# kaspanet/rusty-kaspa

Hardware: AMD Instinct MI355X
Metric: sig-verifies/sec (higher is better)
Workload: dtype u256; 1 GPU; schnorr-verify-1M; tuples_per_gpu=1048576, invalid_permille=0, parallelism=single

## Files before the change

### rusty_kaspa_amd/csrc/kv_secp_device.h

```cpp
#ifndef KV_SECP_DEVICE_H
#define KV_SECP_DEVICE_H

#ifndef KV_HOST_TEST
#include <hip/hip_runtime.h>
#endif
#include <stdint.h>

namespace kv {

#ifdef KV_GROUP_INLINE
#define KV_GROUP_ATTR inline
#else
#define KV_GROUP_ATTR __noinline__
#endif
#if defined(KV_GROUP_INLINE) || defined(KV_DOUBLE_INLINE)
#define KV_DOUBLE_ATTR inline
#else
#define KV_DOUBLE_ATTR __noinline__
#endif

typedef uint64_t u64;
typedef uint32_t u32;
typedef unsigned __int128 u128;


struct fe {
  u64 n[4];
};

#define KV_P0 0xFFFFFFFEFFFFFC2FULL
#define KV_P1 0xFFFFFFFFFFFFFFFFULL
#define KV_PC 0x1000003D1ULL

__device__ __forceinline__ u64 addc(u64 a, u64 b, u64 &carry) {
  u128 t = (u128)a + b + carry;
  carry = (u64)(t >> 64);
  return (u64)t;
}

__device__ __forceinline__ u64 subb(u64 a, u64 b, u64 &borrow) {
  u128 t = (u128)a - b - borrow;
  borrow = (u64)(t >> 64) & 1;
  return (u64)t;
}

__device__ __forceinline__ void fe_norm_once(fe &a) {
  u64 ge = (a.n[3] == KV_P1) & (a.n[2] == KV_P1) & (a.n[1] == KV_P1) &
           (a.n[0] >= KV_P0);
  u64 mask = 0 - ge;
  u64 borrow = 0;
  a.n[0] = subb(a.n[0], KV_P0 & mask, borrow);
  a.n[1] = subb(a.n[1], KV_P1 & mask, borrow);
  a.n[2] = subb(a.n[2], KV_P1 & mask, borrow);
  a.n[3] = subb(a.n[3], KV_P1 & mask, borrow);
}

__device__ __forceinline__ void fe_mul_inner(u64 t[8], const u64 *an, const u64 *bn) {
#pragma unroll
  for (int i = 0; i < 8; i++) t[i] = 0;
#pragma unroll
  for (int i = 0; i < 4; i++) {
    u64 carry = 0;
#pragma unroll
    for (int j = 0; j < 4; j++) {
      u128 cur = (u128)an[i] * bn[j] + t[i + j] + carry;
      t[i + j] = (u64)cur;
      carry = (u64)(cur >> 64);
    }
    t[i + 4] = carry;
  }
}

__device__ __forceinline__ void fe_reduce8(fe &r, const u64 t[8]) {
  u128 c = (u128)t[0] + (u128)t[4] * KV_PC;
  u64 s0 = (u64)c;
  c = (c >> 64) + t[1] + (u128)t[5] * KV_PC;
  u64 s1 = (u64)c;
  c = (c >> 64) + t[2] + (u128)t[6] * KV_PC;
  u64 s2 = (u64)c;
  c = (c >> 64) + t[3] + (u128)t[7] * KV_PC;
  u64 s3 = (u64)c;
  u64 s4 = (u64)(c >> 64);
  c = (u128)s0 + (u128)s4 * KV_PC;
  r.n[0] = (u64)c;
  c = (c >> 64) + s1;
  r.n[1] = (u64)c;
  c = (c >> 64) + s2;
  r.n[2] = (u64)c;
  c = (c >> 64) + s3;
  r.n[3] = (u64)c;
  if ((u64)(c >> 64)) {
    c = (u128)r.n[0] + KV_PC;
    r.n[0] = (u64)c;
    u64 cc = (u64)(c >> 64);
    r.n[1] += cc;
  }
  fe_norm_once(r);
}

__device__ __forceinline__ void fe_mul(fe &r, const fe &a, const fe &b) {
  u64 t[8];
  fe_mul_inner(t, a.n, b.n);
  fe_reduce8(r, t);
}


#define KV26_M ((u32)0x3FFFFFF)
#define KV26_R0 ((u64)0x3D10)

struct fe26 {
#ifdef KV_FE26_ALIGN
  alignas(16) u32 l[10];
#else
  u32 l[10];
#endif
};

#ifdef KV_HOST_TEST
#include <assert.h>
#define KV26_CHECK_MUL_IN(a)                                                   \
  do {                                                                         \
    for (int _i = 0; _i < 10; _i++) assert((a).l[_i] <= (1u << 30));           \
  } while (0)
#else
#define KV26_CHECK_MUL_IN(a)
#endif

__device__ __forceinline__ void fe26_reduce19(fe26 &r, const u64 t[19]) {
  u32 u[11];
  u64 c = t[9] >> 26;
#pragma unroll
  for (int k = 0; k < 9; k++) {
    u64 d = t[k + 10] + c;
    u[k] = (u32)d & KV26_M;
    c = d >> 26;
  }
  u[9] = (u32)c & KV26_M;
  u[10] = (u32)(c >> 26);
  u64 W = ((u64)u[9] << 10) + (u64)u[10] * KV26_R0 + ((u64)u[10] << 36);
  u32 w0 = (u32)W & KV26_M, w1 = (u32)(W >> 26);
  u64 cc = 0;
#pragma unroll
  for (int k = 0; k < 10; k++) {
    u64 d = (k == 9 ? (t[9] & KV26_M) : t[k]) + cc + (u64)u[k] * KV26_R0;
    if (k >= 1) d += (u64)u[k - 1] << 10;
    if (k == 0) d += (u64)w0 * KV26_R0;
    if (k == 1) d += ((u64)w0 << 10) + (u64)w1 * KV26_R0;
    if (k == 2) d += (u64)w1 << 10;
    r.l[k] = (u32)d & KV26_M;
    cc = d >> 26;
  }
#ifdef KV_HOST_TEST
  assert(u[10] <= (1u << 8) && W < ((u64)1 << 45) && cc < (1u << 15));
#endif
  u32 x = (r.l[9] >> 22) + ((u32)cc << 4);
  r.l[9] &= 0x3FFFFF;
  r.l[0] += x * 977u;
  r.l[1] += (x << 6) + (r.l[0] >> 26);
  r.l[0] &= KV26_M;
  r.l[2] += r.l[1] >> 26;
  r.l[1] &= KV26_M;
}

__device__ __forceinline__ void fe26_mul_inner(u64 t[19], const fe26 &a,
                                               const fe26 &b) {
  KV26_CHECK_MUL_IN(a);
  KV26_CHECK_MUL_IN(b);
#pragma unroll
  for (int k = 0; k < 19; k++) t[k] = 0;
#pragma unroll
  for (int i = 0; i < 10; i++)
#pragma unroll
    for (int j = 0; j < 10; j++) t[i + j] += (u64)a.l[i] * b.l[j];

}

__device__ __forceinline__ void fe26_sqr_inner(u64 t[19], const fe26 &a) {
  KV26_CHECK_MUL_IN(a);
  u32 d[9];
#pragma unroll
  for (int i = 0; i < 9; i++) d[i] = a.l[i] << 1;
#pragma unroll
  for (int k = 0; k < 19; k++) t[k] = 0;
#pragma unroll
  for (int i = 0; i < 10; i++) {
    t[2 * i] += (u64)a.l[i] * a.l[i];
#pragma unroll
    for (int j = i + 1; j < 10; j++) t[i + j] += (u64)d[i] * a.l[j];
  }
}

__device__ __forceinline__ void fe26_mul(fe26 &r, const fe26 &a, const fe26 &b) {
  u64 t[19];
  fe26_mul_inner(t, a, b);
  fe26_reduce19(r, t);
}

__device__ __forceinline__ void fe26_sqr(fe26 &r, const fe26 &a) {
  u64 t[19];
  fe26_sqr_inner(t, a);
  fe26_reduce19(r, t);
}

__device__ __forceinline__ void fe26_add(fe26 &r, const fe26 &a, const fe26 &b) {
#pragma unroll
  for (int i = 0; i < 10; i++) r.l[i] = a.l[i] + b.l[i];
}

__device__ __forceinline__ void fe26_neg(fe26 &r, const fe26 &a, u32 m) {
  r.l[0] = (u32)(0x3FFFC2FUL * 2 * (m + 1)) - a.l[0];
  r.l[1] = (u32)(0x3FFFFBFUL * 2 * (m + 1)) - a.l[1];
#pragma unroll
  for (int i = 2; i < 9; i++) r.l[i] = (u32)(0x3FFFFFFUL * 2 * (m + 1)) - a.l[i];
  r.l[9] = (u32)(0x3FFFFFUL * 2 * (m + 1)) - a.l[9];
}

__device__ __forceinline__ void fe26_mul_int(fe26 &r, u32 k) {
#pragma unroll
  for (int i = 0; i < 10; i++) r.l[i] *= k;
}

__device__ __forceinline__ void fe26_cmov(fe26 &r, const fe26 &a, u32 cond) {
  u32 mask = 0 - cond;
#pragma unroll
  for (int i = 0; i < 10; i++) r.l[i] = (r.l[i] & ~mask) | (a.l[i] & mask);
}

__device__ __forceinline__ void fe26_norm_weak(fe26 &a) {
  u32 c = 0;
#pragma unroll
  for (int i = 0; i < 10; i++) {
    u32 d = a.l[i] + c;
    a.l[i] = d & KV26_M;
    c = d >> 26;
  }
  a.l[0] += c * (u32)KV26_R0;
  a.l[1] += c << 10;
  u32 x = a.l[9] >> 22;
  a.l[9] &= 0x3FFFFF;
  a.l[0] += x * 977u;
  a.l[1] += x << 6;
}

__device__ __forceinline__ void fe26_normalize(fe26 &a) {
  fe26_norm_weak(a);
#pragma unroll 1
  for (int pass = 0; pass < 3; pass++) {
    u32 c = 0;
#pragma unroll
    for (int i = 0; i < 10; i++) {
      u32 d = a.l[i] + c;
      a.l[i] = d & KV26_M;
      c = d >> 26;
    }
    u32 x = (a.l[9] >> 22) | (c << 4);
    a.l[9] &= 0x3FFFFF;
    a.l[0] += x * 977u;
    a.l[1] += x << 6;
  }
  u32 t[10];
  u64 d = (u64)a.l[0] + 977u;
  t[0] = (u32)(d & KV26_M);
  d = (d >> 26) + a.l[1] + (1u << 6);
  t[1] = (u32)(d & KV26_M);
#pragma unroll
  for (int i = 2; i < 10; i++) {
    d = (d >> 26) + a.l[i];
    t[i] = (u32)(d & KV26_M);
  }
  u32 ge = (u32)(t[9] >> 22) & 1;
  t[9] &= 0x3FFFFF;
  u32 mask = 0 - ge;
#pragma unroll
  for (int i = 0; i < 10; i++) a.l[i] = (a.l[i] & ~mask) | (t[i] & mask);
}

__device__ __forceinline__ int fe26_is_zero(const fe26 &a) {
  fe26 t = a;
  fe26_normalize(t);
  u32 z = 0;
#pragma unroll
  for (int i = 0; i < 10; i++) z |= t.l[i];
  return z == 0;
}

__device__ __forceinline__ int fe26_eq(const fe26 &a, const fe26 &b) {
  fe26 ta = a, tb = b;
  fe26_normalize(ta);
  fe26_normalize(tb);
  u32 d = 0;
#pragma unroll
  for (int i = 0; i < 10; i++) d |= ta.l[i] ^ tb.l[i];
  return d == 0;
}

__device__ __forceinline__ int fe26_normalizes_to_zero(const fe26 &a) {
#ifdef KV_HOST_TEST
  for (int _i = 0; _i < 10; _i++) assert(a.l[_i] < (1u << 31));
#endif
  u32 l[10];
  u32 c = 0;
#pragma unroll
  for (int i = 0; i < 10; i++) {
    u32 d = a.l[i] + c;
    l[i] = d & KV26_M;
    c = d >> 26;
  }
  u32 x = l[9] >> 22;
  l[9] &= 0x3FFFFF;
  l[0] += c * (u32)KV26_R0 + x * 977u;
  l[1] += (c << 10) + (x << 6) + (l[0] >> 26);
  l[0] &= KV26_M;
  l[2] += l[1] >> 26;
  l[1] &= KV26_M;
  u32 z0 = l[0] | l[1] | l[2] | l[9];
  u32 z1 = (l[0] ^ 0x3D0u) & (l[1] ^ 0x40u) & l[2] & (l[9] ^ 0x3C00000u);
#pragma unroll
  for (int i = 3; i < 9; i++) {
    z0 |= l[i];
    z1 &= l[i];
  }
  return (z0 == 0) | (z1 == KV26_M);
}

__device__ __forceinline__ void fe26_from_fe(fe26 &r, const fe &a) {
#pragma unroll
  for (int i = 0; i < 10; i++) {
    int bit = 26 * i;
    int w = bit >> 6, sh = bit & 63;
    u64 v = a.n[w] >> sh;
    if (sh > 38 && w < 3) v |= a.n[w + 1] << (64 - sh);
    r.l[i] = (u32)(v & KV26_M);
  }
  r.l[9] &= 0x3FFFFF;
}

__device__ __forceinline__ void fe26_to_fe(fe &r, const fe26 &a) {
  r.n[0] = (u64)a.l[0] | ((u64)a.l[1] << 26) | ((u64)a.l[2] << 52);
  r.n[1] = ((u64)a.l[2] >> 12) | ((u64)a.l[3] << 14) | ((u64)a.l[4] << 40);
  r.n[2] = ((u64)a.l[4] >> 24) | ((u64)a.l[5] << 2) | ((u64)a.l[6] << 28) |
           ((u64)a.l[7] << 54);
  r.n[3] = ((u64)a.l[7] >> 10) | ((u64)a.l[8] << 16) | ((u64)a.l[9] << 42);
}


struct sc {
  u64 d[4];
};

#define KV_N0 0xBFD25E8CD0364141ULL
#define KV_N1 0xBAAEDCE6AF48A03BULL
#define KV_N2 0xFFFFFFFFFFFFFFFEULL
#define KV_N3 0xFFFFFFFFFFFFFFFFULL
#define KV_NC0 0x402DA1732FC9BEBFULL
#define KV_NC1 0x4551231950B75FC4ULL
#define KV_NC2 1ULL

__device__ __forceinline__ int sc_gte_n(const sc &a) {
  if (a.d[3] > KV_N3) return 1;
  if (a.d[3] < KV_N3) return 0;
  if (a.d[2] > KV_N2) return 1;
  if (a.d[2] < KV_N2) return 0;
  if (a.d[1] > KV_N1) return 1;
  if (a.d[1] < KV_N1) return 0;
  return a.d[0] >= KV_N0;
}

__device__ __forceinline__ void sc_sub_n(sc &a) {
  u64 borrow = 0;
  a.d[0] = subb(a.d[0], KV_N0, borrow);
  a.d[1] = subb(a.d[1], KV_N1, borrow);
  a.d[2] = subb(a.d[2], KV_N2, borrow);
  a.d[3] = subb(a.d[3], KV_N3, borrow);
}

__device__ __forceinline__ int sc_is_zero(const sc &a) {
  return (a.d[0] | a.d[1] | a.d[2] | a.d[3]) == 0;
}

__device__ __forceinline__ int sc_from_be(sc &r, const uint8_t b[32]) {
#pragma unroll
  for (int i = 0; i < 4; i++) {
    u64 w = 0;
#pragma unroll
    for (int j = 0; j < 8; j++) w = (w << 8) | b[8 * (3 - i) + j];
    r.d[i] = w;
  }
  int ov = sc_gte_n(r);
  if (ov) sc_sub_n(r);
  return ov;
}

__device__ __forceinline__ void sc_neg(sc &r, const sc &a) {
  u64 is_zero = sc_is_zero(a);
  u64 borrow = 0;
  r.d[0] = subb(KV_N0, a.d[0], borrow);
  r.d[1] = subb(KV_N1, a.d[1], borrow);
  r.d[2] = subb(KV_N2, a.d[2], borrow);
  r.d[3] = subb(KV_N3, a.d[3], borrow);
  u64 mask = 0 - is_zero;
  r.d[0] &= ~mask;
  r.d[1] &= ~mask;
  r.d[2] &= ~mask;
  r.d[3] &= ~mask;
}

__device__ inline void sc_reduce8(sc &r, const u64 tin[8]) {
  const u64 NC[3] = {KV_NC0, KV_NC1, KV_NC2};
  u64 s[7] = {tin[0], tin[1], tin[2], tin[3], 0, 0, 0};
  for (int i = 0; i < 4; i++) {
    u64 carry = 0;
    for (int j = 0; j < 3; j++) {
      u64 lo = tin[4 + i] * NC[j];
      u64 hi = __umul64hi(tin[4 + i], NC[j]);
      u64 c = 0;
      s[i + j] = addc(s[i + j], lo, c);
      u64 c2 = 0;
      s[i + j] = addc(s[i + j], carry, c2);
      carry = hi + c + c2;
    }
    u64 c = 0;
    s[i + 3] = addc(s[i + 3], carry, c);
    for (int k = i + 4; k < 7 && c; k++) s[k] = addc(s[k], 0, c);
  }
  u64 u[5] = {s[0], s[1], s[2], s[3], 0};
  for (int i = 0; i < 3; i++) {
    u64 carry = 0;
    for (int j = 0; j < 3; j++) {
      int pos = i + j;
      u64 lo = s[4 + i] * NC[j];
      u64 hi = __umul64hi(s[4 + i], NC[j]);
      u64 c = 0;
      u[pos] = addc(u[pos], lo, c);
      u64 c2 = 0;
      u[pos] = addc(u[pos], carry, c2);
      carry = hi + c + c2;
    }
    if (i + 3 < 5) {
      u64 c = 0;
      u[i + 3] = addc(u[i + 3], carry, c);
      for (int k = i + 4; k < 5 && c; k++) u[k] = addc(u[k], 0, c);
    }
  }
  u64 w[4] = {u[0], u[1], u[2], u[3]};
  {
    u64 carry = 0;
    for (int j = 0; j < 3; j++) {
      u64 lo = u[4] * NC[j];
      u64 hi = __umul64hi(u[4], NC[j]);
      u64 c = 0;
      w[j] = addc(w[j], lo, c);
      u64 c2 = 0;
      w[j] = addc(w[j], carry, c2);
      carry = hi + c + c2;
    }
    u64 c = 0;
    w[3] = addc(w[3], carry, c);
    if (c) {
      u64 cc = 0;
      w[0] = addc(w[0], NC[0], cc);
      w[1] = addc(w[1], NC[1], cc);
      w[2] = addc(w[2], NC[2], cc);
      w[3] = addc(w[3], 0, cc);
    }
  }
  r.d[0] = w[0]; r.d[1] = w[1]; r.d[2] = w[2]; r.d[3] = w[3];
  while (sc_gte_n(r)) sc_sub_n(r);
}

__device__ inline void sc_mul(sc &r, const sc &a, const sc &b) {
  u64 t[8];
  fe_mul_inner(t, a.d, b.d);
  sc_reduce8(r, t);
}

__device__ KV_GROUP_ATTR void sc_sqrn(sc &r, int n) {
#pragma unroll 1
  for (int i = 0; i < n; i++) sc_mul(r, r, r);
}

__device__ KV_GROUP_ATTR void sc_inv(sc &r, const sc &a) {
  static const uint8_t WIN[33] = {14, 11, 10, 10, 14, 13, 12, 14, 6,  10, 15,
                                  4,  8,  10, 0,  3,  11, 11, 15, 13, 2,  5,
                                  14, 8,  12, 13, 0,  3,  6,  4,  1,  3,  15};
  sc tab[16];
  tab[0] = {{1, 0, 0, 0}};
  tab[1] = a;
#pragma unroll 1
  for (int i = 2; i < 16; i++) sc_mul(tab[i], tab[i - 1], a);
  sc x6, x12, x24, t;
  const sc &x3 = tab[7], &x4 = tab[15];
  t = x3;
  sc_sqrn(t, 3);
  sc_mul(x6, t, x3);
  t = x6;
  sc_sqrn(t, 6);
  sc_mul(x12, t, x6);
  t = x12;
  sc_sqrn(t, 12);
  sc_mul(x24, t, x12);
  t = x24;
  sc_sqrn(t, 24);
  sc_mul(t, t, x24);
  sc x48 = t;
  sc_sqrn(t, 48);
  sc_mul(t, t, x48);
  sc_sqrn(t, 24);
  sc_mul(t, t, x24);
  sc_sqrn(t, 4);
  sc_mul(t, t, x4);
#pragma unroll 1
  for (int i = 0; i < 33; i++) {
    sc_sqrn(t, 4);
    sc m;
    sc_mul(m, t, tab[WIN[i]]);
    t = m;
  }
  r = t;
}


__device__ KV_GROUP_ATTR void fe26_sqrn(fe26 &r, int n) {
#pragma unroll 1
  for (int i = 0; i < n; i++) fe26_sqr(r, r);
}

__device__ KV_GROUP_ATTR void fe26_chain223(fe26 &x223, fe26 &x22, fe26 &x2,
                                            fe26 &x3, const fe26 &a) {
  fe26 t, x11, x44, x88;
  fe26_sqr(t, a);
  fe26_mul(x2, t, a);
  fe26_sqr(t, x2);
  fe26_mul(x3, t, a);
  t = x3;
  fe26_sqrn(t, 3);
  fe26_mul(t, t, x3);
  fe26_sqrn(t, 3);
  fe26_mul(t, t, x3);
  fe26_sqrn(t, 2);
  fe26_mul(x11, t, x2);
  t = x11;
  fe26_sqrn(t, 11);
  fe26_mul(x22, t, x11);
  t = x22;
  fe26_sqrn(t, 22);
  fe26_mul(x44, t, x22);
  t = x44;
  fe26_sqrn(t, 44);
  fe26_mul(x88, t, x44);
  t = x88;
  fe26_sqrn(t, 88);
  fe26_mul(t, t, x88);
  fe26_sqrn(t, 44);
  fe26_mul(t, t, x44);
  fe26_sqrn(t, 3);
  fe26_mul(x223, t, x3);
}

__device__ inline void fe26_inv(fe26 &r, const fe26 &a) {
  fe26 x223, x22, x2, x3, t;
  fe26_chain223(x223, x22, x2, x3, a);
  t = x223;
  fe26_sqrn(t, 23);
  fe26_mul(t, t, x22);
  fe26_sqrn(t, 5);
  fe26_mul(t, t, a);
  fe26_sqrn(t, 3);
  fe26_mul(t, t, x2);
  fe26_sqrn(t, 2);
  fe26_mul(r, t, a);
}

__device__ inline int fe26_sqrt(fe26 &r, const fe26 &a) {
  fe26 x223, x22, x2, x3, t, chk;
  fe26_chain223(x223, x22, x2, x3, a);
  t = x223;
  fe26_sqrn(t, 23);
  fe26_mul(t, t, x22);
  fe26_sqrn(t, 6);
  fe26_mul(t, t, x2);
  fe26_sqrn(t, 2);
  fe26_sqr(chk, t);
  r = t;
  fe26 aa = a;
  return fe26_eq(chk, aa);
}


struct ge {
  fe26 x, y;
};

struct gej {
  fe26 x, y, z;
};

__device__ __forceinline__ void fe26_set_int(fe26 &r, u32 v) {
  r.l[0] = v;
#pragma unroll
  for (int i = 1; i < 10; i++) r.l[i] = 0;
}

__device__ __forceinline__ void gej_set_infinity(gej &r) {
  fe26_set_int(r.x, 1);
  fe26_set_int(r.y, 1);
  fe26_set_int(r.z, 0);
}

__device__ __forceinline__ int gej_is_infinity(const gej &a) {
  return fe26_normalizes_to_zero(a.z);
}

__device__ __forceinline__ void gej_double_impl(gej &r, const gej &a) {
  fe26 A, B, C, D, E, F, t, x4, y2;
  fe26_sqr(A, a.x);
  fe26_sqr(B, a.y);
  fe26_sqr(C, B);
  x4 = a.x;
  fe26_mul_int(x4, 4);
  fe26_mul(D, x4, B);
  E = A;
  fe26_mul_int(E, 3);
  fe26_sqr(F, E);
  fe26 nx, ny, nz, nD;
  fe26_neg(nD, D, 2);
  fe26_add(nx, F, nD);
  fe26_add(nx, nx, nD);
  fe26_norm_weak(nx);
  fe26 nnx;
  fe26_neg(nnx, nx, 2);
  fe26_add(t, D, nnx);
  fe26_mul(t, E, t);
  fe26 C8;
  C8 = C;
  fe26_mul_int(C8, 8);
  fe26 nC8;
  fe26_neg(nC8, C8, 16);
  fe26_add(ny, t, nC8);
  fe26_norm_weak(ny);
  fe26_add(y2, a.y, a.y);
  fe26_mul(nz, y2, a.z);
  r.x = nx;
  r.y = ny;
  r.z = nz;
}

__device__ KV_DOUBLE_ATTR void gej_double(gej &r, const gej &a) {
  gej_double_impl(r, a);
}

__device__ KV_GROUP_ATTR void gej_double4(gej &r, const gej &a) {
  gej t;
  gej_double_impl(t, a);
  gej_double_impl(r, t);
  gej_double_impl(t, r);
  gej_double_impl(r, t);
}

__device__ __forceinline__ void gej_cmov(gej &r, const gej &a, u64 cond) {
  u32 c = (u32)(cond & 1);
  fe26_cmov(r.x, a.x, c);
  fe26_cmov(r.y, a.y, c);
  fe26_cmov(r.z, a.z, c);
}

template <bool ZR>
__device__ __forceinline__ void gej_add_ge_core(gej &r, fe26 &zr, const gej &a,
                                                const ge &b) {
  u64 a_inf = (u64)fe26_normalizes_to_zero(a.z);
  fe26 z1z1, u2, s2, h, hh, i, j, rr, v, t;
  fe26_sqr(z1z1, a.z);
  fe26_mul(s2, b.y, a.z);
  fe26_mul(u2, b.x, z1z1);
  fe26_mul(s2, s2, z1z1);
  fe26 nX, nY;
  fe26_neg(nX, a.x, 2);
  fe26_neg(nY, a.y, 2);
  fe26_add(h, u2, nX);
  fe26_add(rr, s2, nY);
  if (!a_inf && fe26_normalizes_to_zero(h)) {
    if (fe26_normalizes_to_zero(rr)) {
      gej t2;
      gej ain = a;
      fe26_norm_weak(ain.x);
      fe26_norm_weak(ain.y);
      fe26_norm_weak(ain.z);
      gej_double_impl(t2, ain);
      r = t2;
      if (ZR) {
        fe26_add(zr, ain.y, ain.y);
        fe26_norm_weak(zr);
      }
    } else {
      gej_set_infinity(r);
      if (ZR) fe26_set_int(zr, 0);
    }
    return;
  }
  if (ZR) {
    fe26_add(zr, h, h);
    fe26_norm_weak(zr);
  }
  fe26 zz;
  fe26_add(zz, a.z, h);
  fe26_sqr(zz, zz);
  fe26_sqr(hh, h);
  i = hh;
  fe26_mul_int(i, 4);
  fe26_mul(j, h, i);
  fe26_mul(v, a.x, i);
  fe26 nx, ny, nz;
  fe26_sqr(nx, rr);
  fe26_mul_int(nx, 4);
  fe26 nj, nv;
  fe26_neg(nj, j, 2);
  fe26_neg(nv, v, 2);
  fe26_add(nx, nx, nj);
  fe26_add(nx, nx, nv);
  fe26_add(nx, nx, nv);
  fe26_norm_weak(nx);
  fe26 nnx;
  fe26_neg(nnx, nx, 2);
  fe26_add(t, v, nnx);
  fe26_mul(t, rr, t);
  fe26_add(t, t, t);
  fe26 y1j;
  fe26_mul(y1j, a.y, j);
  fe26_add(y1j, y1j, y1j);
  fe26 ny1j;
  fe26_neg(ny1j, y1j, 4);
  fe26_add(ny, t, ny1j);
  fe26_norm_weak(ny);
  fe26 nzz, nhh;
  fe26_neg(nzz, z1z1, 2);
  fe26_neg(nhh, hh, 2);
  fe26_add(nz, zz, nzz);
  fe26_add(nz, nz, nhh);
  fe26_norm_weak(nz);
  fe26 one;
  fe26_set_int(one, 1);
  u32 ci = (u32)(a_inf & 1);
  fe26_cmov(nx, b.x, ci);
  fe26_cmov(ny, b.y, ci);
  fe26_cmov(nz, one, ci);
  r.x = nx;
  r.y = ny;
  r.z = nz;
}

__device__ __forceinline__ void gej_add_ge_impl(gej &r, const gej &a, const ge &b) {
  fe26 unused;
  gej_add_ge_core<false>(r, unused, a, b);
}

__device__ KV_GROUP_ATTR void gej_add_ge(gej &r, const gej &a, const ge &b) {
  gej_add_ge_impl(r, a, b);
}

__device__ KV_GROUP_ATTR void gej_add_ge_zr(gej &r, fe26 &zr, const gej &a,
                                            const ge &b) {
  gej_add_ge_core<true>(r, zr, a, b);
}

__device__ KV_GROUP_ATTR void gej_add(gej &r, const gej &a, const gej &b) {
  u64 a_inf = (u64)fe26_normalizes_to_zero(a.z);
  fe26 z1z1, z2z2, u1, u2, s1, s2, h, i, j, rr, v, t;
  fe26_sqr(z1z1, a.z);
  fe26_sqr(z2z2, b.z);
  fe26_mul(u1, a.x, z2z2);
  fe26_mul(u2, b.x, z1z1);
  fe26_mul(s1, a.y, b.z);
  fe26_mul(s1, s1, z2z2);
  fe26_mul(s2, b.y, a.z);
  fe26_mul(s2, s2, z1z1);
  fe26 nu1, ns1;
  fe26_neg(nu1, u1, 2);
  fe26_neg(ns1, s1, 2);
  fe26_add(h, u2, nu1);
  fe26_add(rr, s2, ns1);
  if (!a_inf && !fe26_normalizes_to_zero(b.z) && fe26_normalizes_to_zero(h)) {
    if (fe26_normalizes_to_zero(rr)) {
      gej t2;
      gej ain = a;
      fe26_norm_weak(ain.x);
      fe26_norm_weak(ain.y);
      fe26_norm_weak(ain.z);
      gej_double_impl(t2, ain);
      r = t2;
    } else {
      gej_set_infinity(r);
    }
    return;
  }
  fe26 zz;
  fe26_add(zz, a.z, b.z);
  fe26_sqr(zz, zz);
  fe26_sqr(i, h);
  fe26_mul_int(i, 4);
  fe26_mul(j, h, i);
  fe26_mul(v, u1, i);
  fe26 nx, ny, nz;
  fe26_sqr(nx, rr);
  fe26_mul_int(nx, 4);
  fe26 nj, nv;
  fe26_neg(nj, j, 2);
  fe26_neg(nv, v, 2);
  fe26_add(nx, nx, nj);
  fe26_add(nx, nx, nv);
  fe26_add(nx, nx, nv);
  fe26_norm_weak(nx);
  fe26 nnx;
  fe26_neg(nnx, nx, 2);
  fe26_add(t, v, nnx);
  fe26_mul(t, rr, t);
  fe26_add(t, t, t);
  fe26 s1j;
  fe26_mul(s1j, s1, j);
  fe26_add(s1j, s1j, s1j);
  fe26 ns1j;
  fe26_neg(ns1j, s1j, 4);
  fe26_add(ny, t, ns1j);
  fe26_norm_weak(ny);
  fe26 nzz1, nzz2;
  fe26_neg(nzz1, z1z1, 2);
  fe26_neg(nzz2, z2z2, 2);
  fe26_add(zz, zz, nzz1);
  fe26_add(zz, zz, nzz2);
  fe26_mul(nz, zz, h);
  u32 ci = (u32)(a_inf & 1);
  fe26_cmov(nx, b.x, ci);
  fe26_cmov(ny, b.y, ci);
  fe26_cmov(nz, b.z, ci);
  r.x = nx;
  r.y = ny;
  r.z = nz;
}

}

#endif
```

### rusty_kaspa_amd/csrc/kv_secp_kernels.hip

```cpp
#include "kv_hash_device.h"
#include "kv_secp_device.h"

namespace kv {

__device__ __constant__ static const uint32_t BIP340_CHALLENGE_MID[8] = {
    0x9cecba11u, 0x23925381u, 0x11679112u, 0xd1627e0fu,
    0x97c87550u, 0x003cc765u, 0x90f61164u, 0x33e9b66au};

enum : uint8_t {
  KVS_VALID = 0,
  KVS_INVALID = 1,
  KVS_BAD_PUBKEY = 2,
  KVS_BAD_SIG = 3,
};

__device__ __forceinline__ void fe_from_be(fe &r, const uint8_t b[32]) {
#pragma unroll
  for (int i = 0; i < 4; i++) {
    u64 w = 0;
#pragma unroll
    for (int j = 0; j < 8; j++) w = (w << 8) | b[8 * (3 - i) + j];
    r.n[i] = w;
  }
}

__device__ __forceinline__ int fe_gte_p_full(const fe &a) {
  return (a.n[3] == KV_P1) & (a.n[2] == KV_P1) & (a.n[1] == KV_P1) &
         (a.n[0] >= KV_P0);
}

__device__ inline int lift_x_parity(ge &P, const uint8_t xb[32], u32 want_odd) {
  fe xu;
  fe_from_be(xu, xb);
  if (fe_gte_p_full(xu)) return 0;
  fe26 x, x3, y2, y;
  fe26_from_fe(x, xu);
  fe26_sqr(x3, x);
  fe26_mul(x3, x3, x);
  fe26 seven;
  fe26_set_int(seven, 7);
  fe26_add(y2, x3, seven);
  if (!fe26_sqrt(y, y2)) return 0;
  fe26_normalize(y);
  fe26 ny;
  fe26_neg(ny, y, 1);
  fe26_cmov(y, ny, (y.l[0] & 1) ^ want_odd);
  P.x = x;
  P.y = y;
  return 1;
}

__device__ inline int lift_x_even(ge &P, const uint8_t xb[32]) {
  return lift_x_parity(P, xb, 0);
}

__device__ inline int parse_compressed(ge &P, const uint8_t pk[33]) {
  if (pk[0] != 0x02 && pk[0] != 0x03) return 0;
  return lift_x_parity(P, pk + 1, pk[0] == 0x03);
}

__device__ __constant__ static const u64 GE_G_X[4] = {
    0x59F2815B16F81798ULL, 0x029BFCDB2DCE28D9ULL, 0x55A06295CE870B07ULL,
    0x79BE667EF9DCBBACULL};
__device__ __constant__ static const u64 GE_G_Y[4] = {
    0x9C47D08FFB10D4B8ULL, 0xFD17B448A6855419ULL, 0x5DA4FBFC0E1108A8ULL,
    0x483ADA7726A3C465ULL};

__device__ ge KV_G_TABLE8[256];
__device__ ge KV_H_TABLE8[256];
__device__ static fe26 KV_G8_X[256];
__device__ static fe26 KV_G8_Y[256];
__device__ static fe26 KV_G8_Z[256];
__device__ static fe26 KV_G8_PREF[256];

struct alignas(64) g16_entry {
  u32 w[16];
};
#define KV_G_JOINT_ENTRIES 65536u
#ifndef KV_HOST_TEST
__device__ g16_entry KV_G_JOINT[KV_G_JOINT_ENTRIES];
#endif

#ifndef KV_NO_G_JOINT
#define KV_G_JOINT_LADDER 1
#endif

__device__ inline void g8_table_fill(ge *tab, fe26 *sx, fe26 *sy, fe26 *sz,
                                     fe26 *pref, const ge &B) {
  gej acc;
  acc.x = B.x;
  acc.y = B.y;
  fe26_set_int(acc.z, 1);
  for (int k = 1; k <= 255; k++) {
    sx[k] = acc.x;
    sy[k] = acc.y;
    sz[k] = acc.z;
    gej t;
    gej_add_ge(t, acc, B);
    acc = t;
  }
  pref[1] = sz[1];
  for (int k = 2; k <= 255; k++) fe26_mul(pref[k], pref[k - 1], sz[k]);
  fe26 inv;
  fe26_inv(inv, pref[255]);
  for (int k = 255; k >= 1; k--) {
    fe26 zi;
    if (k > 1) {
      fe26_mul(zi, inv, pref[k - 1]);
      fe26_mul(inv, inv, sz[k]);
    } else {
      zi = inv;
    }
    fe26 zi2, zi3;
    ge e;
    fe26_sqr(zi2, zi);
    fe26_mul(zi3, zi2, zi);
    fe26_mul(e.x, sx[k], zi2);
    fe26_mul(e.y, sy[k], zi3);
    fe26_normalize(e.x);
    fe26_normalize(e.y);
    tab[k] = e;
  }
  tab[0] = tab[1];
}

__device__ inline void g8_h_base(ge &H, const ge &G) {
  gej acc;
  acc.x = G.x;
  acc.y = G.y;
  fe26_set_int(acc.z, 1);
  for (int k = 0; k < 128; k++) {
    gej t;
    gej_double(t, acc);
    acc = t;
  }
  fe26 zi, zi2, zi3;
  fe26_inv(zi, acc.z);
  fe26_sqr(zi2, zi);
  fe26_mul(zi3, zi2, zi);
  fe26_mul(H.x, acc.x, zi2);
  fe26_mul(H.y, acc.y, zi3);
  fe26_normalize(H.x);
  fe26_normalize(H.y);
}

__device__ __forceinline__ void g16_pack_fe(u32 w[8], const fe26 &a) {
  fe f;
  fe26_to_fe(f, a);
#pragma unroll
  for (int i = 0; i < 4; i++) {
    w[2 * i] = (u32)f.n[i];
    w[2 * i + 1] = (u32)(f.n[i] >> 32);
  }
}

__device__ __forceinline__ void g16_unpack_fe(fe26 &r, const u32 w[8]) {
#pragma unroll
  for (int i = 0; i < 10; i++) {
    int bit = 26 * i;
    int k = bit >> 5, sh = bit & 31;
    u32 v = w[k] >> sh;
    if (sh > 6 && k < 7) v |= w[k + 1] << (32 - sh);
    r.l[i] = v & KV26_M;
  }
}

__device__ __forceinline__ void g16_unpack(ge &e, const g16_entry &t) {
  g16_unpack_fe(e.x, t.w);
  g16_unpack_fe(e.y, t.w + 8);
}

__device__ inline void g16_build_entry(g16_entry &out, u32 idx, const ge *g8,
                                       const ge *h8) {
  u32 lo = idx & 255, hi = (idx >> 8) & 255;
  ge e;
  if (hi == 0) {
    e = g8[lo];
  } else if (lo == 0) {
    e = h8[hi];
  } else {
    gej a, s;
    a.x = g8[lo].x;
    a.y = g8[lo].y;
    fe26_set_int(a.z, 1);
    gej_add_ge(s, a, h8[hi]);
    fe26 zi, zi2, zi3;
    fe26_inv(zi, s.z);
    fe26_sqr(zi2, zi);
    fe26_mul(zi3, zi2, zi);
    fe26_mul(e.x, s.x, zi2);
    fe26_mul(e.y, s.y, zi3);
    fe26_normalize(e.x);
    fe26_normalize(e.y);
  }
  g16_pack_fe(out.w, e.x);
  g16_pack_fe(out.w + 8, e.y);
}

extern "C" __global__ void kv_ec_table_init_kernel() {
  if (threadIdx.x != 0 || blockIdx.x != 0) return;
  ge G, H;
  {
    fe gx, gy;
#pragma unroll
    for (int i = 0; i < 4; i++) {
      gx.n[i] = GE_G_X[i];
      gy.n[i] = GE_G_Y[i];
    }
    fe26_from_fe(G.x, gx);
    fe26_from_fe(G.y, gy);
  }
  g8_table_fill(KV_G_TABLE8, KV_G8_X, KV_G8_Y, KV_G8_Z, KV_G8_PREF, G);
  g8_h_base(H, G);
  g8_table_fill(KV_H_TABLE8, KV_G8_X, KV_G8_Y, KV_G8_Z, KV_G8_PREF, H);
}

#ifndef KV_HOST_TEST
extern "C" __global__ void __launch_bounds__(256) kv_g_joint_init_kernel() {
  u32 idx = blockIdx.x * blockDim.x + threadIdx.x;
  if (idx >= KV_G_JOINT_ENTRIES) return;
  g16_entry e;
  g16_build_entry(e, idx, KV_G_TABLE8, KV_H_TABLE8);
  KV_G_JOINT[idx] = e;
}

__device__ __forceinline__ void g16_fetch(ge &e, u32 idx) {
  g16_unpack(e, KV_G_JOINT[idx & (KV_G_JOINT_ENTRIES - 1)]);
}
#else
static inline void g16_fetch(ge &e, u32 idx) {
  static ge base;
  static bool have = false;
  static fe26 sx[256], sy[256], sz[256], pref[256];
  bool same = have;
  for (int i = 0; same && i < 10; i++)
    same = base.x.l[i] == KV_G_TABLE8[1].x.l[i] &&
           base.y.l[i] == KV_G_TABLE8[1].y.l[i];
  if (!same) {
    ge H;
    base = KV_G_TABLE8[1];
    g8_h_base(H, base);
    g8_table_fill(KV_H_TABLE8, sx, sy, sz, pref, H);
    have = true;
  }
  g16_entry t;
  g16_build_entry(t, idx & (KV_G_JOINT_ENTRIES - 1), KV_G_TABLE8, KV_H_TABLE8);
  g16_unpack(e, t);
}
#endif


__device__ __constant__ static const u64 GLV_BETA[4] = {
    0xc1396c28719501eeULL, 0x9cf0497512f58995ULL, 0x6e64479eac3434e9ULL,
    0x7ae96a2b657c0710ULL};
__device__ __constant__ static const u64 GLV_G1[4] = {
    0xe893209a45dbb031ULL, 0x3daa8a1471e8ca7fULL, 0xe86c90e49284eb15ULL,
    0x3086d221a7d46bcdULL};
__device__ __constant__ static const u64 GLV_G2[4] = {
    0x1571b4ae8ac47f71ULL, 0x221208ac9df506c6ULL, 0x6f547fa90abfe4c4ULL,
    0xe4437ed6010e8828ULL};
__device__ __constant__ static const u64 GLV_A1[4] = {
    0xe86c90e49284eb15ULL, 0x3086d221a7d46bcdULL, 0x0000000000000000ULL,
    0x0000000000000000ULL};
__device__ __constant__ static const u64 GLV_B1[4] = {
    0x90ab8056f5401b3dULL, 0x1bbc8129fef177d7ULL, 0xffffffffffffffffULL,
    0xffffffffffffffffULL};
__device__ __constant__ static const u64 GLV_A2[4] = {
    0x57c1108d9d44cfd8ULL, 0x14ca50f7a8e2f3f6ULL, 0x0000000000000001ULL,
    0x0000000000000000ULL};
__device__ __constant__ static const u64 GLV_B2[4] = {
    0xe86c90e49284eb15ULL, 0x3086d221a7d46bcdULL, 0x0000000000000000ULL,
    0x0000000000000000ULL};

__device__ __forceinline__ void mul_low256(u64 r[4], const u64 a[4], const u64 b[4]) {
  u64 t[8];
  fe_mul_inner(t, a, b);
#pragma unroll
  for (int i = 0; i < 4; i++) r[i] = t[i];
}

__device__ __forceinline__ void mul_shift384(u64 c[2], const u64 g[4], const u64 k[4]) {
  u64 t[8];
  fe_mul_inner(t, g, k);
  c[0] = t[6];
  c[1] = t[7];
}

struct glv_half {
  u64 d[3];
  u64 neg;
};

__device__ inline void glv_split(const sc &k, glv_half &h1, glv_half &h2) {
  u64 c1[4] = {0, 0, 0, 0}, c2[4] = {0, 0, 0, 0};
  mul_shift384(c1, GLV_G1, k.d);
  mul_shift384(c2, GLV_G2, k.d);
  u64 t1[4], t2[4], k1[4], k2[4];
  mul_low256(t1, c1, GLV_A1);
  mul_low256(t2, c2, GLV_A2);
  {
    u64 borrow = 0;
#pragma unroll
    for (int i = 0; i < 4; i++) k1[i] = subb(k.d[i], t1[i], borrow);
    borrow = 0;
#pragma unroll
    for (int i = 0; i < 4; i++) k1[i] = subb(k1[i], t2[i], borrow);
  }
  mul_low256(t1, c1, GLV_B1);
  mul_low256(t2, c2, GLV_B2);
  {
    u64 carry = 0;
#pragma unroll
    for (int i = 0; i < 4; i++) t1[i] = addc(t1[i], t2[i], carry);
    u64 borrow = 0;
#pragma unroll
    for (int i = 0; i < 4; i++) k2[i] = subb(0, t1[i], borrow);
  }
  u64 n1 = k1[3] >> 63, n2 = k2[3] >> 63;
  u64 carry = 1;
#pragma unroll
  for (int i = 0; i < 4; i++) {
    u64 v = n1 ? ~k1[i] : k1[i];
    u128 s = (u128)v + (n1 ? carry : 0);
    if (n1) {
      k1[i] = (u64)s;
      carry = (u64)(s >> 64);
    } else {
      k1[i] = v;
    }
  }
  carry = 1;
#pragma unroll
  for (int i = 0; i < 4; i++) {
    u64 v = n2 ? ~k2[i] : k2[i];
    u128 s = (u128)v + (n2 ? carry : 0);
    if (n2) {
      k2[i] = (u64)s;
      carry = (u64)(s >> 64);
    } else {
      k2[i] = v;
    }
  }
  h1.d[0] = k1[0]; h1.d[1] = k1[1]; h1.d[2] = k1[2]; h1.neg = n1;
  h2.d[0] = k2[0]; h2.d[1] = k2[1]; h2.d[2] = k2[2]; h2.neg = n2;
}

__device__ __forceinline__ u64 glv_digit(const glv_half &h, int w) {
  int bit = w * 4;
  int limb = bit >> 6, sh = bit & 63;
  u64 v = h.d[limb] >> sh;
  if (sh > 60 && limb < 2) v |= h.d[limb + 1] << (64 - sh);
  return v & 15;
}

__device__ __forceinline__ u64 glv_digit8(const glv_half &h, int w) {
  int bit = w * 4;
  int limb = bit >> 6, sh = bit & 63;
  u64 v = h.d[limb] >> sh;
  if (sh > 56 && limb < 2) v |= h.d[limb + 1] << (64 - sh);
  return v & 255;
}

#ifndef KV_NO_SIGNED_PTAB
#define KV_SIGNED_PTAB 1
#endif

#ifdef KV_SIGNED_PTAB
__device__ __forceinline__ void glv_recode_signed(const glv_half &h,
                                                  int8_t dig[33]) {
  u64 carry = 0;
#pragma unroll 1
  for (int w = 0; w < 33; w++) {
    u64 v = glv_digit(h, w) + carry;
    carry = v > 8;
    dig[w] = (int8_t)((long long)v - (long long)(carry << 4));
  }
}
#endif

#ifdef KV_SIGNED_PTAB
#define KV_PTAB_MAX 8
#else
#define KV_PTAB_MAX 15
#endif

struct ladder_consts {
  fe26 beta;
  fe26 zg2;
  fe26 zg3;
#ifndef KV_G_JOINT_LADDER
  fe26 bzg2;
#endif
};

#ifdef KV_G_JOINT_LADDER
struct g_digits {
  u32 idx;
};
#else
struct g_digits {
  u64 d1, n1, d2, n2;
};
#endif

__device__ inline void ecmult_ptab_build(ge *ptab, ladder_consts &lc, fe26 &zg,
                                         const ge &P) {
  fe26 zr[KV_PTAB_MAX + 1];
  gej acc;
  acc.x = P.x;
  acc.y = P.y;
  fe26_set_int(acc.z, 1);
#pragma unroll 1
  for (int k = 2; k <= KV_PTAB_MAX; k++) {
    gej t;
    gej_add_ge_zr(t, zr[k], acc, P);
    acc = t;
    ptab[k].x = acc.x;
    ptab[k].y = acc.y;
  }
  zg = acc.z;
  fe26 m = zr[KV_PTAB_MAX];
#pragma unroll 1
  for (int k = KV_PTAB_MAX - 1; k >= 2; k--) {
    fe26 m2, m3;
    fe26_sqr(m2, m);
    fe26_mul(m3, m2, m);
    fe26_mul(ptab[k].x, ptab[k].x, m2);
    fe26_mul(ptab[k].y, ptab[k].y, m3);
    if (k > 2) fe26_mul(m, m, zr[k]);
  }
  fe26_sqr(lc.zg2, zg);
  fe26_mul(lc.zg3, lc.zg2, zg);
  fe26_mul(ptab[1].x, P.x, lc.zg2);
  fe26_mul(ptab[1].y, P.y, lc.zg3);
  ptab[0] = ptab[1];
}

template <bool IS_G, bool PHI>
__device__ __forceinline__ void ladder_entry(ge &e, const ge &tab,
                                             const ladder_consts &lc, u64 neg) {
  e = tab;
#ifndef KV_G_JOINT_LADDER
  if (IS_G) {
    fe26 mx, my;
    fe26_mul(mx, e.x, PHI ? lc.bzg2 : lc.zg2);
    fe26_mul(my, e.y, lc.zg3);
    e.x = mx;
    e.y = my;
  } else
#endif
  if (PHI) {
    fe26 bx;
    fe26_mul(bx, e.x, lc.beta);
    e.x = bx;
  }
  fe26 ny;
  fe26_neg(ny, e.y, 2);
  fe26_cmov(e.y, ny, (u32)neg);
}

template <bool IS_G, bool PHI>
__device__ __forceinline__ void ladder_add(gej &R, const ge &tab,
                                           const ladder_consts &lc, u64 digit,
                                           u64 neg) {
  ge e;
  gej t;
  ladder_entry<IS_G, PHI>(e, tab, lc, neg);
  gej_add_ge_impl(t, R, e);
  gej_cmov(R, t, (u64)(digit != 0));
}

__device__ __forceinline__ void ladder_add_g(gej &R, const ladder_consts &lc,
                                             const g_digits &g) {
#ifdef KV_G_JOINT_LADDER
  ge e, m;
  gej t;
  g16_fetch(e, g.idx);
  fe26_mul(m.x, e.x, lc.zg2);
  fe26_mul(m.y, e.y, lc.zg3);
  gej_add_ge_impl(t, R, m);
  gej_cmov(R, t, (u64)(g.idx != 0));
#else
  ladder_add<true, false>(R, KV_G_TABLE8[g.d1], lc, g.d1, g.n1);
  ladder_add<true, true>(R, KV_G_TABLE8[g.d2], lc, g.d2, g.n2);
#endif
}

template <bool DOUBLE, bool G_ACTIVE>
__device__ __forceinline__ void gej_window_impl(gej &R, const ge *ptab,
                                                const ladder_consts &lc,
                                                const g_digits &g, u64 dp1,
                                                u64 np1, u64 dp2, u64 np2) {
  if (DOUBLE) {
    gej t;
    gej_double_impl(t, R);
    gej_double_impl(R, t);
    gej_double_impl(t, R);
    gej_double_impl(R, t);
  }
  if (G_ACTIVE) ladder_add_g(R, lc, g);
  ladder_add<false, false>(R, ptab[dp1], lc, dp1, np1);
  ladder_add<false, true>(R, ptab[dp2], lc, dp2, np2);
}

__device__ KV_GROUP_ATTR void gej_window_step(gej &R, const ge *ptab,
                                              const ladder_consts &lc,
                                              u64 g_active, g_digits g, u64 dp1,
                                              u64 np1, u64 dp2, u64 np2) {
  if (g_active)
    gej_window_impl<true, true>(R, ptab, lc, g, dp1, np1, dp2, np2);
  else
    gej_window_impl<true, false>(R, ptab, lc, g, dp1, np1, dp2, np2);
}

__device__ KV_GROUP_ATTR void gej_window_first(gej &R, const ge *ptab,
                                               const ladder_consts &lc,
#ifndef KV_G_JOINT_LADDER
                                               g_digits g,
#endif
                                               u64 dp1, u64 np1, u64 dp2,
                                               u64 np2) {
  gej_set_infinity(R);
#ifdef KV_G_JOINT_LADDER
  gej_window_impl<false, false>(R, ptab, lc, g_digits{0}, dp1, np1, dp2, np2);
#else
  gej_window_impl<false, true>(R, ptab, lc, g, dp1, np1, dp2, np2);
#endif
}

#ifndef KV_NO_PAIR_WINDOWS
#define KV_PAIR_WINDOWS 1
#endif

#ifdef KV_PAIR_WINDOWS
__device__ __forceinline__ void gej_window_pair_impl(
    gej &R, const ge *ptab, const ladder_consts &lc, const g_digits &g,
    u64 hp1, u64 hn1, u64 hp2, u64 hn2,
    u64 lp1, u64 ln1, u64 lp2, u64 ln2 ) {
  gej_window_impl<true, false>(R, ptab, lc, g, hp1, hn1, hp2, hn2);
  gej_window_impl<true, true>(R, ptab, lc, g, lp1, ln1, lp2, ln2);
}

__device__ KV_GROUP_ATTR void gej_window_step2(gej &R, const ge *ptab,
                                               const ladder_consts &lc,
                                               g_digits g, u64 hp1, u64 hn1,
                                               u64 hp2, u64 hn2, u64 lp1,
                                               u64 ln1, u64 lp2, u64 ln2) {
  gej_window_pair_impl(R, ptab, lc, g, hp1, hn1, hp2, hn2, lp1, ln1, lp2, ln2);
}

#ifdef KV_QUAD_WINDOWS
__device__ KV_GROUP_ATTR void gej_window_step4(gej &R, const ge *ptab,
                                               const ladder_consts &lc,
                                               g_digits ga, g_digits gb,
                                               const u64 a[8], const u64 b[8]) {
  gej_window_pair_impl(R, ptab, lc, ga, a[0], a[1], a[2], a[3], a[4], a[5],
                       a[6], a[7]);
  gej_window_pair_impl(R, ptab, lc, gb, b[0], b[1], b[2], b[3], b[4], b[5],
                       b[6], b[7]);
}
#endif
#endif

__device__ inline void ecmult_double(gej &R, const sc &gs, const sc &ps,
                                     const ge &P) {
  glv_half p1h, p2h;
  glv_split(ps, p1h, p2h);
#ifndef KV_G_JOINT_LADDER
  glv_half g1h, g2h;
  glv_split(gs, g1h, g2h);
#endif
  ge ptab[KV_PTAB_MAX + 1];
  ladder_consts lc;
  fe26 zg;
  ecmult_ptab_build(ptab, lc, zg, P);
#ifdef KV_SIGNED_PTAB
  int8_t dp1[33], dp2[33];
  glv_recode_signed(p1h, dp1);
  glv_recode_signed(p2h, dp2);
#endif
  {
    fe bu;
#pragma unroll
    for (int i = 0; i < 4; i++) bu.n[i] = GLV_BETA[i];
    fe26_from_fe(lc.beta, bu);
#ifndef KV_G_JOINT_LADDER
    fe26_mul(lc.bzg2, lc.beta, lc.zg2);
#endif
  }
#ifdef KV_SIGNED_PTAB
#define KV_DP1(w) ((u64)(dp1[w] < 0 ? -dp1[w] : dp1[w]))
#define KV_DN1(w) ((u64)((dp1[w] < 0) ^ (int)p1h.neg))
#define KV_DP2(w) ((u64)(dp2[w] < 0 ? -dp2[w] : dp2[w]))
#define KV_DN2(w) ((u64)((dp2[w] < 0) ^ (int)p2h.neg))
#else
#define KV_DP1(w) glv_digit(p1h, w)
#define KV_DN1(w) (p1h.neg)
#define KV_DP2(w) glv_digit(p2h, w)
#define KV_DN2(w) (p2h.neg)
#endif
#ifdef KV_G_JOINT_LADDER
#define KV_GD(w)                                                               \
  (g_digits{(u32)((gs.d[2 + ((w) >> 4)] >> (((w) & 14) << 2)) & 255) << 8 |    \
            (u32)((gs.d[(w) >> 4] >> (((w) & 14) << 2)) & 255)})
#else
#define KV_GD(w)                                                               \
  (g_digits{glv_digit8(g1h, w), g1h.neg, glv_digit8(g2h, w), g2h.neg})
#endif
  gej_window_first(R, ptab, lc,
#ifndef KV_G_JOINT_LADDER
                   KV_GD(32),
#endif
                   KV_DP1(32), KV_DN1(32), KV_DP2(32), KV_DN2(32));
#if defined(KV_QUAD_WINDOWS)
#pragma unroll 1
  for (int w = 31; w >= 3; w -= 4) {
    u64 a[8] = {KV_DP1(w), KV_DN1(w), KV_DP2(w), KV_DN2(w),
                KV_DP1(w - 1), KV_DN1(w - 1), KV_DP2(w - 1), KV_DN2(w - 1)};
    u64 b[8] = {KV_DP1(w - 2), KV_DN1(w - 2), KV_DP2(w - 2), KV_DN2(w - 2),
                KV_DP1(w - 3), KV_DN1(w - 3), KV_DP2(w - 3), KV_DN2(w - 3)};
    gej_window_step4(R, ptab, lc, KV_GD(w - 1), KV_GD(w - 3), a, b);
  }
#elif defined(KV_PAIR_WINDOWS)
#pragma unroll 1
  for (int w = 31; w >= 1; w -= 2) {
    gej_window_step2(R, ptab, lc, KV_GD(w - 1),
                     KV_DP1(w), KV_DN1(w), KV_DP2(w), KV_DN2(w),
                     KV_DP1(w - 1), KV_DN1(w - 1), KV_DP2(w - 1), KV_DN2(w - 1));
  }
#else
#pragma unroll 1
  for (int w = 31; w >= 0; w--) {
    u64 g_active = (w & 1) == 0;
    gej_window_step(R, ptab, lc, g_active, KV_GD(w & ~1),
                    KV_DP1(w), KV_DN1(w), KV_DP2(w), KV_DN2(w));
  }
#endif
#undef KV_GD
#undef KV_DP1
#undef KV_DN1
#undef KV_DP2
#undef KV_DN2
  fe26 rz;
  fe26_mul(rz, R.z, zg);
  R.z = rz;
}

__device__ inline uint8_t schnorr_ladder_one(gej &R, fe26 &rx, const uint8_t *rb,
                                             const uint8_t *sb, const uint8_t *pkb,
                                             const uint8_t *msg) {
  ge P;
  if (!lift_x_even(P, pkb)) return KVS_BAD_PUBKEY;
  fe rxu;
  fe_from_be(rxu, rb);
  if (fe_gte_p_full(rxu)) return KVS_INVALID;
  fe26_from_fe(rx, rxu);
  sc s;
  if (sc_from_be(s, sb)) return KVS_INVALID;
  uint8_t eh[32];
  sha256_tagged96(BIP340_CHALLENGE_MID, rb, pkb, msg, eh);
  sc e, ne;
  sc_from_be(e, eh);
  sc_neg(ne, e);
  ecmult_double(R, s, ne, P);
  return 0;
}

__device__ __forceinline__ uint8_t schnorr_affine_verdict(const gej &R,
                                                          const fe26 &zi,
                                                          const fe26 &rx) {
  fe26 zi2, zi3, xa, ya;
  fe26_sqr(zi2, zi);
  fe26_mul(zi3, zi2, zi);
  fe26_mul(xa, R.x, zi2);
  fe26_mul(ya, R.y, zi3);
  fe26_normalize(ya);
  if (ya.l[0] & 1) return KVS_INVALID;
  return fe26_eq(xa, rx) ? KVS_VALID : KVS_INVALID;
}

__device__ inline uint8_t schnorr_verify_one(const uint8_t *rb, const uint8_t *sb,
                                             const uint8_t *pkb, const uint8_t *msg) {
  gej R;
  fe26 rx;
  uint8_t pre = schnorr_ladder_one(R, rx, rb, sb, pkb, msg);
  if (pre) return pre;
  if (gej_is_infinity(R)) return KVS_INVALID;
  fe26 zi;
  fe26_inv(zi, R.z);
  return schnorr_affine_verdict(R, zi, rx);
}

#ifndef KV_FINISH_K
#define KV_FINISH_K 16
#endif

__device__ __forceinline__ void fin_load26(fe26 &v, const u32 *__restrict__ limbs,
                                           unsigned long long n, int coord,
                                           unsigned long long i) {
#pragma unroll
  for (int j = 0; j < 10; j++) v.l[j] = limbs[(unsigned long long)(10 * coord + j) * n + i];
}

__device__ __forceinline__ void fin_load_z(fe26 &z, const u32 *__restrict__ limbs,
                                           unsigned long long n,
                                           unsigned long long i, uint8_t code) {
  fe26 one;
  fe26_set_int(one, 1);
  fin_load26(z, limbs, n, 2, i);
  fe26_cmov(z, one, (u32)(code != 0));
}

__device__ inline void schnorr_finish_lane(uint8_t st[KV_FINISH_K],
                                           const u32 *__restrict__ limbs,
                                           const uint8_t *__restrict__ pre,
                                           const uint8_t *__restrict__ tuples,
                                           unsigned long long n,
                                           unsigned long long first,
                                           unsigned long long step) {
  fe26 pref[KV_FINISH_K];
  fe26 acc, one;
  fe26_set_int(acc, 1);
  fe26_set_int(one, 1);
#pragma unroll 1
  for (int m = 0; m < KV_FINISH_K; m++) {
    unsigned long long i = first + (unsigned long long)m * step;
    u32 inr = i < n;
    unsigned long long ii = inr ? i : n - 1;
    uint8_t code = inr ? pre[ii] : (uint8_t)KVS_INVALID;
    fe26 z;
    fin_load_z(z, limbs, n, ii, code);
    u32 inf = (u32)fe26_normalizes_to_zero(z);
    fe26_cmov(z, one, inf);
    st[m] = inf ? (uint8_t)KVS_INVALID : code;
    pref[m] = acc;
    fe26_mul(acc, acc, z);
  }
  fe26 inv;
  fe26_inv(inv, acc);
#pragma unroll 1
  for (int m = KV_FINISH_K - 1; m >= 0; m--) {
    unsigned long long i = first + (unsigned long long)m * step;
    unsigned long long ii = i < n ? i : n - 1;
    uint8_t code = st[m];
    fe26 z, zi;
    fin_load_z(z, limbs, n, ii, code);
    fe26_mul(zi, inv, pref[m]);
    fe26_mul(inv, inv, z);
    if (code == 0) {
      gej R;
      fin_load26(R.x, limbs, n, 0, ii);
      fin_load26(R.y, limbs, n, 1, ii);
      fe rxu;
      fe_from_be(rxu, tuples + ii * 128);
      fe26 rx;
      fe26_from_fe(rx, rxu);
      st[m] = schnorr_affine_verdict(R, zi, rx);
    }
  }
}

#ifndef KV_LB
#define KV_LB __launch_bounds__(256, 3)
#endif
extern "C" __global__ void KV_LB kv_schnorr_verify_kernel(const uint8_t *__restrict__ tuples,
                                                    unsigned long long n,
                                                    unsigned long long *__restrict__ bitmap,
                                                    uint8_t *__restrict__ status) {
  unsigned long long i = (unsigned long long)blockIdx.x * blockDim.x + threadIdx.x;
  int valid = 0;
  if (i < n) {
    const uint8_t *t = tuples + i * 128;
    uint8_t st = schnorr_verify_one(t, t + 32, t + 64, t + 96);
    if (status) status[i] = st;
    valid = (st == KVS_VALID);
  }
  unsigned long long mask = __ballot(valid);
  if ((threadIdx.x & 63) == 0) {
    unsigned long long word = i / 64;
    if (i < n) bitmap[word] = mask;
  }
}

#ifndef KV_HOST_TEST
extern "C" __global__ void KV_LB kv_schnorr_ladder_kernel(const uint8_t *__restrict__ tuples,
                                                    unsigned long long n,
                                                    u32 *__restrict__ limbs,
                                                    uint8_t *__restrict__ pre) {
  unsigned long long i = (unsigned long long)blockIdx.x * blockDim.x + threadIdx.x;
  if (i >= n) return;
  const uint8_t *t = tuples + i * 128;
  gej R;
  fe26 rx;
  uint8_t st = schnorr_ladder_one(R, rx, t, t + 32, t + 64, t + 96);
  pre[i] = st;
  if (st) return;
#pragma unroll
  for (int j = 0; j < 10; j++) {
    limbs[(unsigned long long)j * n + i] = R.x.l[j];
    limbs[(unsigned long long)(10 + j) * n + i] = R.y.l[j];
    limbs[(unsigned long long)(20 + j) * n + i] = R.z.l[j];
  }
}

extern "C" __global__ void __launch_bounds__(64)
kv_schnorr_finish_kernel(const uint8_t *__restrict__ tuples, unsigned long long n,
                         const u32 *__restrict__ limbs,
                         const uint8_t *__restrict__ pre, unsigned long long T,
                         unsigned long long *__restrict__ bitmap,
                         uint8_t *__restrict__ status) {
  unsigned long long t = (unsigned long long)blockIdx.x * blockDim.x + threadIdx.x;
  uint8_t st[KV_FINISH_K];
  schnorr_finish_lane(st, limbs, pre, tuples, n, t, T);
#pragma unroll 1
  for (int m = 0; m < KV_FINISH_K; m++) {
    unsigned long long i = (unsigned long long)m * T + t;
    int valid = 0;
    if (i < n) {
      if (status) status[i] = st[m];
      valid = (st[m] == KVS_VALID);
    }
    unsigned long long mask = __ballot(valid);
    if ((threadIdx.x & 63) == 0 && i < n) bitmap[i / 64] = mask;
  }
}
#endif


__device__ inline uint8_t ecdsa_verify_one(const uint8_t *rb, const uint8_t *sb,
                                           const uint8_t *pk33, const uint8_t *msg) {
  ge P;
  if (!parse_compressed(P, pk33)) return KVS_BAD_PUBKEY;
  sc r, s;
  if (sc_from_be(r, rb)) return KVS_BAD_SIG;
  if (sc_from_be(s, sb)) return KVS_BAD_SIG;
  if (sc_is_zero(r) || sc_is_zero(s)) return KVS_INVALID;
  static const u64 NHALF[4] = {0xDFE92F46681B20A0ULL, 0x5D576E7357A4501DULL,
                               0xFFFFFFFFFFFFFFFFULL, 0x7FFFFFFFFFFFFFFFULL};
  int high = 0;
  for (int i = 3; i >= 0; i--) {
    if (s.d[i] > NHALF[i]) { high = 1; break; }
    if (s.d[i] < NHALF[i]) break;
  }
  if (high) return KVS_INVALID;
  sc z;
  sc_from_be(z, msg);
  sc w, u1, u2;
  sc_inv(w, s);
  sc_mul(u1, z, w);
  sc_mul(u2, r, w);
  gej R;
  ecmult_double(R, u1, u2, P);
  if (gej_is_infinity(R)) return KVS_INVALID;
  fe26 z2;
  fe26_sqr(z2, R.z);
  fe rf;
  rf.n[0] = r.d[0];
  rf.n[1] = r.d[1];
  rf.n[2] = r.d[2];
  rf.n[3] = r.d[3];
  fe26 rf26, t;
  fe26_from_fe(rf26, rf);
  fe26_mul(t, rf26, z2);
  if (fe26_eq(t, R.x)) return KVS_VALID;
  u64 carry = 0;
  fe rn;
  rn.n[0] = addc(rf.n[0], KV_N0, carry);
  rn.n[1] = addc(rf.n[1], KV_N1, carry);
  rn.n[2] = addc(rf.n[2], KV_N2, carry);
  rn.n[3] = addc(rf.n[3], KV_N3, carry);
  if (!carry && !fe_gte_p_full(rn)) {
    fe26 rn26;
    fe26_from_fe(rn26, rn);
    fe26_mul(t, rn26, z2);
    if (fe26_eq(t, R.x)) return KVS_VALID;
  }
  return KVS_INVALID;
}

extern "C" __global__ void KV_LB kv_ecdsa_verify_kernel(const uint8_t *__restrict__ tuples,
                                                  unsigned long long n,
                                                  unsigned long long *__restrict__ bitmap,
                                                  uint8_t *__restrict__ status) {
  unsigned long long i = (unsigned long long)blockIdx.x * blockDim.x + threadIdx.x;
  int valid = 0;
  if (i < n) {
    const uint8_t *t = tuples + i * 132;
    uint8_t st = ecdsa_verify_one(t, t + 32, t + 64, t + 97);
    if (status) status[i] = st;
    valid = (st == KVS_VALID);
  }
  unsigned long long mask = __ballot(valid);
  if ((threadIdx.x & 63) == 0 && i < n) bitmap[i / 64] = mask;
}

}
```

Before: 64.24 million verifies/s.

## Restructure 26-bit field reduction folding and copy ladder state into locals

Rewrites fe26_reduce19 so the high limbs are folded into the low limbs with 32-bit multiply-accumulates by constants, which are forced into scalar registers, instead of a serial carry chain followed by a second fold. This is meant to shorten the dependent carry chain and cut 64-bit shift and multiply work in every field multiply. The noinline window functions also copy the gej accumulator into a local before working on it and write it back afterwards, so the compiler can keep it in registers rather than going through a pointer. The new reduction carries different bounds, checked only in host-test asserts, and the copies could add register pressure.

New measurement: 72.79 million verifies/s (median of 6 runs). 1.13x the previous value.

```diff
diff --git a/rusty_kaspa_amd/csrc/kv_secp_device.h b/rusty_kaspa_amd/csrc/kv_secp_device.h
--- a/rusty_kaspa_amd/csrc/kv_secp_device.h
+++ b/rusty_kaspa_amd/csrc/kv_secp_device.h
@@ -126,32 +126,67 @@
 #define KV26_CHECK_MUL_IN(a)
 #endif
 
+__device__ __forceinline__ u32 kv26_mulc(u32 c) {
+#ifndef KV_HOST_TEST
+  asm("" : "+s"(c));
+#endif
+  return c;
+}
+
 __device__ __forceinline__ void fe26_reduce19(fe26 &r, const u64 t[19]) {
-  u32 u[11];
-  u64 c = t[9] >> 26;
-#pragma unroll
-  for (int k = 0; k < 9; k++) {
-    u64 d = t[k + 10] + c;
-    u[k] = (u32)d & KV26_M;
-    c = d >> 26;
-  }
-  u[9] = (u32)c & KV26_M;
-  u[10] = (u32)(c >> 26);
-  u64 W = ((u64)u[9] << 10) + (u64)u[10] * KV26_R0 + ((u64)u[10] << 36);
-  u32 w0 = (u32)W & KV26_M, w1 = (u32)(W >> 26);
+  const u32 c6 = kv26_mulc(1u << 6), c10 = kv26_mulc(1u << 10),
+            c16 = kv26_mulc(1u << 16), r0 = kv26_mulc((u32)KV26_R0),
+            r6 = kv26_mulc((u32)KV26_R0 << 6),
+            r16 = kv26_mulc((u32)KV26_R0 << 16);
+  u64 s[19];
+#pragma unroll
+  for (int k = 0; k < 19; k++) {
+    s[k] = t[k];
+#ifdef KV_HOST_TEST
+    assert(s[k] <= (u64)(k < 10 ? k + 1 : 19 - k) << 60);
+#endif
+  }
+#pragma unroll
+  for (int j = 9; j < 18; j++) {
+    u32 h = (u32)(s[j] >> 32);
+    s[j] = (u32)s[j];
+    s[j + 1] += (u64)h * c6;
+#ifdef KV_HOST_TEST
+    assert(s[j + 1] <= ((u64)(18 - j) << 60) + ((u64)1 << 38));
+#endif
+  }
+  u32 h18 = (u32)(s[18] >> 32);
+  s[18] = (u32)s[18];
+  s[9] += (u64)h18 * r6;
+  s[0] += (u64)h18 * r16;
+  s[2] += h18;
+#pragma unroll
+  for (int j = 10; j < 19; j++) {
+    u32 lo = (u32)s[j];
+    s[j - 10] += (u64)lo * r0;
+    s[j - 9] += (u64)lo * c10;
+  }
+  u32 h9 = (u32)(s[9] >> 32);
+#ifdef KV_HOST_TEST
+  assert(h18 < (1u << 29) && s[9] < ((u64)1 << 50) && h9 < (1u << 18));
+#endif
+  s[9] = (u32)s[9];
+  s[0] += (u64)h9 * r6;
+  s[1] += (u64)h9 * c16;
   u64 cc = 0;
 #pragma unroll
   for (int k = 0; k < 10; k++) {
-    u64 d = (k == 9 ? (t[9] & KV26_M) : t[k]) + cc + (u64)u[k] * KV26_R0;
-    if (k >= 1) d += (u64)u[k - 1] << 10;
-    if (k == 0) d += (u64)w0 * KV26_R0;
-    if (k == 1) d += ((u64)w0 << 10) + (u64)w1 * KV26_R0;
-    if (k == 2) d += (u64)w1 << 10;
+#ifdef KV_HOST_TEST
+    assert(k == 9 ? s[9] < ((u64)1 << 32)
+                  : s[k] <= ((u64)(k + 1) << 60) + ((u64)1 << 59));
+    assert(cc < ((u64)1 << 38));
+#endif
+    u64 d = s[k] + cc;
     r.l[k] = (u32)d & KV26_M;
     cc = d >> 26;
   }
 #ifdef KV_HOST_TEST
-  assert(u[10] <= (1u << 8) && W < ((u64)1 << 45) && cc < (1u << 15));
+  assert(cc < (1u << 13));
 #endif
   u32 x = (r.l[9] >> 22) + ((u32)cc << 4);
   r.l[9] &= 0x3FFFFF;
diff --git a/rusty_kaspa_amd/csrc/kv_secp_kernels.hip b/rusty_kaspa_amd/csrc/kv_secp_kernels.hip
--- a/rusty_kaspa_amd/csrc/kv_secp_kernels.hip
+++ b/rusty_kaspa_amd/csrc/kv_secp_kernels.hip
@@ -520,12 +520,14 @@
 #endif
                                                u64 dp1, u64 np1, u64 dp2,
                                                u64 np2) {
-  gej_set_infinity(R);
+  gej r;
+  gej_set_infinity(r);
 #ifdef KV_G_JOINT_LADDER
-  gej_window_impl<false, false>(R, ptab, lc, g_digits{0}, dp1, np1, dp2, np2);
+  gej_window_impl<false, false>(r, ptab, lc, g_digits{0}, dp1, np1, dp2, np2);
 #else
-  gej_window_impl<false, true>(R, ptab, lc, g, dp1, np1, dp2, np2);
-#endif
+  gej_window_impl<false, true>(r, ptab, lc, g, dp1, np1, dp2, np2);
+#endif
+  R = r;
 }
 
 #ifndef KV_NO_PAIR_WINDOWS
@@ -546,7 +548,9 @@
                                                g_digits g, u64 hp1, u64 hn1,
                                                u64 hp2, u64 hn2, u64 lp1,
                                                u64 ln1, u64 lp2, u64 ln2) {
-  gej_window_pair_impl(R, ptab, lc, g, hp1, hn1, hp2, hn2, lp1, ln1, lp2, ln2);
+  gej r = R;
+  gej_window_pair_impl(r, ptab, lc, g, hp1, hn1, hp2, hn2, lp1, ln1, lp2, ln2);
+  R = r;
 }
 
 #ifdef KV_QUAD_WINDOWS
```
